# marekvinkler/NTrace

Measured on AMD Instinct MI355X. Metric: Mrays/sec (primary + 8xAO) on Crytek Sponza, higher is better.
Workload: dtype f32

## Files before the change

### ntrace_amd/csrc/ntr_api.cpp

```cpp

#include <hip/hip_runtime.h>

#include <cstdarg>
#include <cstdio>
#include <cstring>
#include <mutex>

#include "ntrace_amd.h"
#include "ntr_internal.h"
#include "compact_bvh.h"
#include "device_scratch.h"
#include "sched_state.h"
#include "trace_kernels.h"
#include "trace_plan.h"

namespace {

thread_local char g_err[512] = "";

}

namespace ntr {

int set_error(int code, const char* fmt, ...)
// ... 91 lines not shown
            if (zk != hipSuccess) return hip_fail(zk, "zero_words launch");
        }
        L->refresh = hs.refresh;
        hint->predicted = false;
        hint->uses++;
        if (hs.useOrder) p.order = hint->order;
        if (L->refresh) {
            const hipError_t ze = ntr_launch_zero_words(hint->cost, orderBlocks, s);
            if (ze != hipSuccess) return hip_fail(ze, "zero_words launch");
            p.cost = hint->cost;
        }
    }

    if (pl.predictable && !(hint && hint->valid) && !p.order) {
        rc = top_table_get(ds, p.nodes, nodesBytes, s, false, &L->predTable);
        if (rc != NTR_OK) return rc;
        rc = predict_scratch_get(ds, s, orderBlocks, &L->predScratch);
        if (rc != NTR_OK) return rc;
        if (L->predScratch) p.order = (hint && pl.hintable) ? hint->order : L->predScratch->order;
        else L->predTable = nullptr;
    }

    L->probeCoherence = !L->predScratch && hint && L->refresh && pl.probeOnRefresh;
    if (L->probeCoherence) {
        rc = top_table_get(ds, p.nodes, nodesBytes, s, false, &L->predTable);
        if (rc != NTR_OK) return rc;
    }
    const unsigned int* word = nullptr;
    if (L->predScratch) word = L->predScratch->classCount + NTR_SCHED_PRED_CLASSES + 2;
    else if (hint && pl.hintable && hint->numBlocks == orderBlocks && hint->order) word = hint->order + orderBlocks + 2;
    const bool routed = pl.coherentRoute == 1 && word != nullptr;
    L->persistentSide = variant == NTR_VARIANT_PERSISTENT || routed;
    L->perraySide = variant != NTR_VARIANT_PERSISTENT || routed;
    if ((pl.minipool && pl.poolKFromDevice) || L->persistentSide) p.poolK = word;

    TraceParams& pp = L->pp = p;
    if (L->persistentSide) {
        rc = counter_set_take(ds, capturing, &pp.counter);
        if (rc != NTR_OK) return rc;
        pp.numBlocks = pl.persistentBlocks; pp.numBlocksIncoherent = pl.numBlocksIncoherent; pp.numBlocksDivergent = pl.numBlocksDivergent;
        pp.fetchThreshold = pl.persistentFetchThreshold;
        pp.shardRays = pl.shardRays;
        if (pp.order) {
            pp.orderBlocks = orderBlocks;
            pp.shardRays = ((orderBlocks + pp.numHeads - 1) / pp.numHeads) * 256;
        }
        pp.routeSkip = routed ? NTR_ROUTE_SKIP_COHERENT : 0;
    }
    if (routed) {
        p.routeSkip = NTR_ROUTE_SKIP_INCOHERENT;
        if (variant == NTR_VARIANT_PERSISTENT) { p.fetchThreshold = pl.perrayFetchThreshold; p.poolKConst = 1; }
    }
    return NTR_OK;
}

static int launch_trace(DeviceState* ds, const Tunables& tun, const TracePlan& pl, const TraceLaunch& L, hipStream_t s, float* seconds,
                        NtrTraceStats* stats)
{
    const TraceParams& p = L.p;
    NtrSchedHint* hint = L.hint;
    const int orderBlocks = pl.orderBlocks;
    StreamEvents<2> ev(s);
    if (seconds) {
        NTR_HIP(ev.create());
        NTR_HIP(hipStreamSynchronize(s));
        NTR_HIP(ev.record(0));
    }
    if (L.predScratch) {
        const hipError_t pe = ntr_launch_predict(p.rays, p.numRays, orderBlocks, L.predTable->table, L.predTable->count, L.predScratch->classCount,
                                                 L.predScratch->classList, (hint && pl.hintable) ? hint->order : L.predScratch->order,
                                                 (hint && pl.hintable) ? hint->order + orderBlocks + 2 : nullptr, pl.minipoolWide, s);
        if (pe != hipSuccess) return hip_fail(pe, "predict launch");
    } else if (L.probeCoherence) {
        const hipError_t ce = ntr_launch_coherence(p.rays, p.numRays, orderBlocks, L.predTable->table, L.predTable->count, hint->order + orderBlocks,
                                                  pl.minipoolWide, s);
        if (ce != hipSuccess) return hip_fail(ce, "coherence launch");
    }
    hipError_t le = hipSuccess;
    if (L.persistentSide) {
        le = ntr_launch_zero_words(L.pp.counter, kPoolHeadsMax * 16, s);
        if (le != hipSuccess) return hip_fail(le, "zero_words launch");
        le = ntr_launch_trace(pl.persistentVariant, &L.pp, pl.persistentBlocks, s);
        if (le != hipSuccess) return hip_fail(le, "trace_bvh launch");
    }
    if (L.perraySide) {
        le = pl.variant == NTR_VARIANT_PERSISTENT ? ntr_launch_trace(NTR_VARIANT_PERRAY_UNIFIED_MINI, &p, pl.perrayBlocks, s)
                                                  : ntr_launch_trace(pl.launchVariant, &p, pl.launchBlocks, s);
        if (le != hipSuccess) return hip_fail(le, "trace_bvh launch");
    }
    if (seconds) NTR_HIP(ev.record(1));
    if (L.refresh) {
        le = ntr_launch_sched_order(hint->cost, orderBlocks, tun.schedClasses, hint->order, 1, s);
        if (le != hipSuccess) return hip_fail(le, "sched_order launch");
        hint->valid = true;
    }
    if (seconds) {
        float ms = 0.0f;
        NTR_HIP(ev.elapsed(0, 1, &ms));
        *seconds = ms * 1e-3f;
        unsigned int st = 0;
        const int rc = status_fetch(ds, s, &st);
        if (rc != NTR_OK) return rc;
        if (st & NTR_STATUS_STACK_OVERFLOW) return set_error(NTR_ERR_OVERFLOW, "trace_bvh: traversal stack overflow");
    }
    if (stats) {
        unsigned long long h[4];
        NTR_HIP(hipMemcpyAsync(h, ds->stats, sizeof(h), hipMemcpyDeviceToHost, s));
        NTR_HIP(hipStreamSynchronize(s));
        stats->numRays = p.numRays;
        stats->numInnerVisits = (int64_t)h[0]; stats->numTriTests = (int64_t)h[1]; stats->numLeafVisits = (int64_t)h[2]; stats->numHits = (int64_t)h[3];
    }
    return NTR_OK;
}

static int trace_impl(const char* kernelName, int32_t numRays, int32_t anyHit, const NtrRay* d_rays,
                      NtrRayResult* d_results, const void* d_nodes, int64_t nodesBytes, const void* d_triWoop,
                      int64_t triWoopBytes, const int32_t* d_triIndex, int32_t layout, uint32_t bvhFlags,
                      void* stream, float* seconds, NtrTraceStats* stats, NtrSchedHint* hint = nullptr)
{
    if (seconds) *seconds = 0.0f;
    if (stats) memset(stats, 0, sizeof(*stats));
    const KernelInfo* k = find_kernel(kernelName);
    if (!k) return set_error(NTR_ERR_UNKNOWN_KERNEL, "unknown kernel '%s'", kernelName ? kernelName : "(null)");
    if (numRays < 0) return set_error(NTR_ERR_INVALID, "ntr_trace_bvh: numRays < 0");
    if (numRays == 0) return NTR_OK;
    if (!d_nodes || !d_triWoop || !d_triIndex)
        return set_error(NTR_ERR_INVALID, "CudaBVHTracer: No BVH!");
    if (layout != k->cfg.bvhLayout)
        return set_error(NTR_ERR_LAYOUT, "CudaBVHTracer: Incorrect BVH layout!");
    if (!d_rays || !d_results) return set_error(NTR_ERR_INVALID, "ntr_trace_bvh: null ray/result buffer");
    int rc = check_nodes_bytes("ntr_trace_bvh", "node buffer size", nodesBytes);
    if (rc != NTR_OK) return rc;
    if (triWoopBytes < 16 || (triWoopBytes % 16) != 0 || triWoopBytes > 0xFFFFFFFFll)
        return set_error(NTR_ERR_INVALID, "ntr_trace_bvh: triWoop buffer size must be a multiple of 16 in [16, 4 GiB)");

    DeviceState* ds = nullptr;
    rc = current_device_state_ready(&ds);
    if (rc != NTR_OK) return rc;
    hipStream_t s = (hipStream_t)stream;

    const Tunables tun = tunables();
    const TraceBatchDesc bd = describe_batch(k, numRays, anyHit, (uint64_t)d_nodes, nodesBytes, (uint64_t)d_triWoop, triWoopBytes, bvhFlags,
                                             stats != nullptr, stream_is_capturing(s), hint != nullptr, ds->numCUs);
    const TracePlan pl = plan_trace(tun, bd);

    TraceLaunch L;
    TraceParams& p = L.p;
    p.numRays = numRays; p.anyHit = anyHit ? 1 : 0; p.rays = d_rays; p.results = d_results; p.bvhFlags = bvhFlags;
    p.nodes = d_nodes; p.woop = d_triWoop; p.triIndex = d_triIndex; p.nodesBytes = (uint32_t)nodesBytes; p.woopBytes = (uint32_t)triWoopBytes;
    p.status = ds->status; p.stats = ds->stats;
    p.numHeads = pl.numHeads; p.chunk = pl.chunk; p.fetchThreshold = pl.fetchThreshold; p.wholeWave = pl.wholeWave; p.prefetchAfter = pl.prefetchAfter;
    p.flatFetch = pl.flatFetch; p.uniformPrologue = pl.uniformPrologue; p.splitSlice = pl.splitSlice; p.leafSwitchBelow = pl.leafSwitchBelow;
    p.octant = pl.octant; p.poolKConst = pl.poolKConst;
    if (stats) NTR_HIP(hipMemsetAsync(ds->stats, 0, 4 * sizeof(unsigned long long), s));

    rc = bind_trace(ds, tun, pl, bd.capturing, nodesBytes, s, hint, &L);
    if (rc != NTR_OK) return rc;
    return launch_trace(ds, tun, pl, L, s, seconds, stats);
}

}

static int env_int(const char* name, int def)
{
    const char* v = getenv(name);
    return (v && *v) ? atoi(v) : def;
}

namespace ntr {
static Tunables g_tun;
static bool g_tunLoaded = false;
static std::mutex g_tunMu;

static void tunables_load_locked()
{
    Tunables t;
    t.chunk = env_int("NTR_TRACE_CHUNK", 64);
    t.fetchThreshold = env_int("NTR_TRACE_FETCH_THRESHOLD", -1);
    t.leafSwitchBelow = env_int("NTR_TRACE_LEAF_SWITCH", -1);
    t.blocksPerCU = env_int("NTR_TRACE_BLOCKS_PER_CU", 7);
    t.blocksPerCUIncoherent = env_int("NTR_TRACE_BLOCKS_PER_CU_INCOHERENT", 3);
    t.blocksPerCUDivergent = env_int("NTR_TRACE_BLOCKS_PER_CU_DIVERGENT", 4);
    t.octant = env_int("NTR_TRACE_OCTANT", 1);
    t.flatFetch = env_int("NTR_TRACE_FLAT_FETCH", 1);
    t.uniformPrologue = env_int("NTR_TRACE_UNIFORM_PROLOGUE", 1);
    t.splitSlice = env_int("NTR_TRACE_SPLIT_SLICE", 8);
    t.wholeWave = env_int("NTR_TRACE_WHOLE_WAVE", 1);
    t.prefetchAfter = env_int("NTR_TRACE_PREFETCH_AFTER", 8);
    t.minipool = env_int("NTR_TRACE_MINIPOOL", -1);
    t.minipoolWide = env_int("NTR_TRACE_MINIPOOL_WIDE", -1);
    t.minipoolThreshold = env_int("NTR_TRACE_MINIPOOL_THRESHOLD", 48);
    t.unified = env_int("NTR_TRACE_UNIFIED", 1);
    t.poolHeads = env_int("NTR_TRACE_POOL_HEADS", 128);
    t.autoHint = env_int("NTR_TRACE_AUTO_HINT", 1);
    t.autoHintMinRays = env_int("NTR_TRACE_AUTO_HINT_MIN_RAYS", 1 << 17);
    t.route = env_int("NTR_TRACE_ROUTE", 1);
    t.persistentHints = env_int("NTR_TRACE_PERSISTENT_HINTS", 1);
    t.predict = env_int("NTR_TRACE_PREDICT", 1);
    t.predictPersistent = env_int("NTR_TRACE_PREDICT_PERSISTENT", 1);
    t.predictDepth = env_int("NTR_TRACE_PREDICT_DEPTH", 9);
    t.predictMinRays = env_int("NTR_TRACE_PREDICT_MIN_RAYS", 1 << 20);
    t.predictMinNodes = env_int("NTR_TRACE_PREDICT_MIN_NODES", 4096);
    t.schedRefreshEvery = env_int("NTR_SCHED_REFRESH_EVERY", 16);
    t.schedClasses = env_int("NTR_SCHED_CLASSES", 32);
    t.lbvhSplit = env_int("NTR_LBVH_SPLIT", 3072);
    t.lbvhAggLds = env_int("NTR_LBVH_AGG_LDS", 1);
    t.lbvhSortItems = env_int("NTR_LBVH_SORT_ITEMS", 0);
    t.lbvhAggStaged = env_int("NTR_LBVH_AGG_STAGED", -1);
    if (t.chunk < 1) t.chunk = 1;
    g_tun = t;
    g_tunLoaded = true;
}

Tunables tunables()
{
    std::lock_guard<std::mutex> lk(g_tunMu);
    if (!g_tunLoaded) tunables_load_locked();
    return g_tun;
}
}

extern "C" int ntr_tunables_reload(void)
{
    std::lock_guard<std::mutex> lk(ntr::g_tunMu);
    ntr::tunables_load_locked();
    return NTR_OK;
}


using namespace ntr;

extern "C" {

const char* ntr_last_error(void) { return g_err; }
int ntr_version(void) { return 100; }

int ntr_device_count(int* count)
{
    if (!count) return set_error(NTR_ERR_INVALID, "ntr_device_count: null argument");
    hipError_t e = hipGetDeviceCount(count);
    if (e != hipSuccess) { *count = 0; return hip_fail(e, "hipGetDeviceCount"); }
    return NTR_OK;
}

int ntr_set_device(int device) { NTR_HIP(hipSetDevice(device)); return NTR_OK; }

int ntr_malloc(void** d_ptr, size_t bytes)
{
    if (!d_ptr) return set_error(NTR_ERR_INVALID, "ntr_malloc: null argument");
    *d_ptr = nullptr;
    if (bytes == 0) return NTR_OK;
    NTR_HIP(hipMalloc(d_ptr, bytes));
    return NTR_OK;
}

int ntr_free(void* d_ptr)
{
    if (d_ptr) NTR_HIP(hipFree(d_ptr));
    return NTR_OK;
}

int ntr_memcpy_h2d(void* d, const void* h, size_t n, void* stream)
{
    if (n == 0) return NTR_OK;
    NTR_HIP(hipMemcpyAsync(d, h, n, hipMemcpyHostToDevice, (hipStream_t)stream));
    NTR_HIP(hipStreamSynchronize((hipStream_t)stream));
    return NTR_OK;
}

int ntr_memcpy_d2h(void* h, const void* d, size_t n, void* stream)
{
    if (n == 0) return NTR_OK;
    NTR_HIP(hipMemcpyAsync(h, d, n, hipMemcpyDeviceToHost, (hipStream_t)stream));
    NTR_HIP(hipStreamSynchronize((hipStream_t)stream));
    return NTR_OK;
}

int ntr_memcpy_d2d(void* dst, const void* src, size_t n, void* stream)
{
    if (n == 0) return NTR_OK;
    NTR_HIP(hipMemcpyAsync(dst, src, n, hipMemcpyDeviceToDevice, (hipStream_t)stream));
    return NTR_OK;
}

int ntr_memset(void* d, int value, size_t n, void* stream)
{
    if (n == 0) return NTR_OK;
    NTR_HIP(hipMemsetAsync(d, value, n, (hipStream_t)stream));
    return NTR_OK;
}

int ntr_stream_synchronize(void* stream)
{
    NTR_HIP(hipStreamSynchronize((hipStream_t)stream));
    return NTR_OK;
}

int ntr_query_config(const char* kernelName, NtrKernelConfig* config)
{
    if (!config) return set_error(NTR_ERR_INVALID, "ntr_query_config: null config");
    const KernelInfo* k = find_kernel(kernelName);
    if (!k) {
        config->bvhLayout = NTR_BVHLayout_Max;
        config->blockWidth = config->blockHeight = config->usePersistentThreads = 0;
        return set_error(NTR_ERR_UNKNOWN_KERNEL, "unknown kernel '%s'", kernelName ? kernelName : "(null)");
    }
    *config = k->cfg;
    return NTR_OK;
}

int ntr_trace_bvh(const char* kernelName, int32_t numRays, int32_t anyHit, const NtrRay* d_rays,
                  NtrRayResult* d_results, const void* d_nodes, int64_t nodesBytes, const void* d_triWoop,
                  int64_t triWoopBytes, const int32_t* d_triIndex, int32_t layout, uint32_t bvhFlags, void* stream,
                  float* seconds)
{
    return trace_impl(kernelName, numRays, anyHit, d_rays, d_results, d_nodes, nodesBytes, d_triWoop, triWoopBytes,
                      d_triIndex, layout, bvhFlags, stream, seconds, nullptr);
}

int ntr_trace_bvh_hinted(const char* kernelName, int32_t numRays, int32_t anyHit, const NtrRay* d_rays,
                         NtrRayResult* d_results, const void* d_nodes, int64_t nodesBytes, const void* d_triWoop,
                         int64_t triWoopBytes, const int32_t* d_triIndex, int32_t layout, uint32_t bvhFlags, void* stream,
                         float* seconds, NtrSchedHint* hint)
{
    return trace_impl(kernelName, numRays, anyHit, d_rays, d_results, d_nodes, nodesBytes, d_triWoop, triWoopBytes,
                      d_triIndex, layout, bvhFlags, stream, seconds, nullptr, hint);
}

int ntr_trace_plan(const char* kernelName, int32_t numRays, int32_t anyHit, uint64_t nodesAddr, int64_t nodesBytes, uint64_t triWoopAddr,
                   int64_t triWoopBytes, uint32_t bvhFlags, int32_t numCUs, int32_t flags, NtrTracePlan* plan)
{
    if (!plan) return set_error(NTR_ERR_INVALID, "ntr_trace_plan: null plan");
    memset(plan, 0, sizeof(*plan));
    const KernelInfo* k = find_kernel(kernelName);
    if (!k) return set_error(NTR_ERR_UNKNOWN_KERNEL, "unknown kernel '%s'", kernelName ? kernelName : "(null)");
    if (numRays < 0 || numCUs < 1 || nodesBytes < 0 || triWoopBytes < 0) return set_error(NTR_ERR_INVALID, "ntr_trace_plan: bad argument");
    const TraceBatchDesc bd = describe_batch(k, numRays, anyHit, nodesAddr, nodesBytes, triWoopAddr, triWoopBytes, bvhFlags,
                                             (flags & NTR_PLAN_FLAG_STATS) != 0, (flags & NTR_PLAN_FLAG_CAPTURING) != 0,
// ... 200 lines not shown
```

### ntrace_amd/csrc/ntr_internal.h

```cpp
#pragma once
#include <hip/hip_runtime.h>

#include "ntrace_amd.h"

namespace ntr {
constexpr int kMaxDevices = 64;

int set_error(int code, const char* fmt, ...) __attribute__((format(printf, 2, 3)));
int hip_fail(hipError_t e, const char* what);

struct Tunables {
    int chunk, fetchThreshold, leafSwitchBelow, blocksPerCU, blocksPerCUIncoherent, blocksPerCUDivergent, poolHeads, octant, unified, flatFetch, uniformPrologue, splitSlice, wholeWave, prefetchAfter, minipool, minipoolThreshold, minipoolWide;
    int autoHint, autoHintMinRays, persistentHints, route, predict, predictPersistent, predictDepth, predictMinRays, predictMinNodes;
    int schedRefreshEvery, schedClasses;
    int lbvhSplit, lbvhAggLds, lbvhAggStaged, lbvhSortItems;
};
Tunables tunables();

bool stream_is_capturing(hipStream_t s);

size_t lbvh_sort_scratch_bytes(int n);
int lbvh_sort_codes(int n, const int32_t* d_tri, const float* d_pos, const float sceneMin[3], const float sceneMax[3], void* scratch,
                    hipStream_t s, const unsigned int** keys, const int** idx, const unsigned int** errWord);
}

extern "C" int ntr_top_table_refresh(const void* d_nodes, int64_t nodesBytes, void* stream);

#define NTR_HIP(call)                                            \
    do {                                                         \
        hipError_t _e = (call);                                  \
        if (_e != hipSuccess) return ::ntr::hip_fail(_e, #call); \
    } while (0)
```

### ntrace_amd/csrc/trace_kernels.h

```cpp
#pragma once
#include <hip/hip_runtime.h>
#include <stdint.h>

#include "ntrace_amd.h"

#ifndef NTR_TRACE_WAVES_PER_BLOCK
#define NTR_TRACE_WAVES_PER_BLOCK 4
#endif
#ifndef NTR_TRACE_MIN_WAVES_PER_SIMD
#define NTR_TRACE_MIN_WAVES_PER_SIMD 1
#endif
#ifndef NTR_TRACE_PERSISTENT_MIN_WAVES_PER_SIMD
#define NTR_TRACE_PERSISTENT_MIN_WAVES_PER_SIMD 1
#endif

#define NTR_VARIANT_PERRAY 0
#define NTR_VARIANT_PERSISTENT 1
#define NTR_VARIANT_PERRAY_STATS 2
#define NTR_VARIANT_PERSISTENT_UNIFIED 5
#define NTR_VARIANT_PERRAY_UNIFIED_W1 6
#define NTR_MINIPOOL_MAX_K 16
#define NTR_VARIANT_PERRAY_UNIFIED_MINI 7

#define NTR_ROUTE_SKIP_COHERENT 1
#define NTR_ROUTE_SKIP_INCOHERENT 2
#define NTR_BATCH_WORD_K(w) ((w) & 0xFFFFu)
#define NTR_BATCH_WORD_INCOHERENT(w) (NTR_BATCH_WORD_K(w) > 1u || ((w) & NTR_BATCH_DIVERGENT) != 0u)

#define NTR_STATUS_STACK_OVERFLOW 1u


namespace ntr {

struct TraceParams {
    int32_t numRays;
    int32_t anyHit;
    const NtrRay* rays;
    NtrRayResult* results;
    const void* nodes;
    const void* woop;
    uint32_t nodesBytes;
    uint32_t woopBytes;
    const int32_t* triIndex;
    int32_t* counter;
    unsigned int* status;
    int32_t chunk;
    int32_t shardRays;
    int32_t numHeads;
    int32_t numBlocks;
    int32_t numBlocksIncoherent;
    int32_t numBlocksDivergent;
    int32_t orderBlocks;
    int32_t fetchThreshold;
    int32_t wholeWave;
    int32_t prefetchAfter;
    uint32_t bvhFlags;
    int32_t leafSwitchBelow;
    int32_t octant;
    int32_t flatFetch;
    int32_t uniformPrologue;
    int32_t splitSlice;
    const unsigned int* order;
    unsigned int* cost;
    unsigned long long* stats;
    const unsigned int* poolK;
    int32_t poolKConst;
    int32_t routeSkip;
};

}

extern "C" hipError_t ntr_launch_trace(int variant, const ntr::TraceParams* p, int numBlocks, hipStream_t stream);
#define NTR_TOP_DEPTH_MAX 10
#define NTR_SCHED_PRED_CLASSES 64
#define NTR_SCHED_PRED_WORDS (NTR_SCHED_PRED_CLASSES + 3)
extern "C" hipError_t ntr_launch_top_table(const void* d_nodes, unsigned int nodesBytes, int depth, void* d_table,
                                           unsigned int* d_tableCount, hipStream_t stream);
extern "C" hipError_t ntr_launch_predict(const void* d_rays, int numRays, int numBlocks, const void* d_table,
                                         const unsigned int* d_tableCount, unsigned int* d_classCount, unsigned int* d_classList,
                                         unsigned int* d_order, unsigned int* d_poolKCopy, int poolKWide, hipStream_t stream);
extern "C" hipError_t ntr_launch_predict_costs(const void* d_rays, int numRays, int numBlocks, const void* d_table,
                                               const unsigned int* d_tableCount, unsigned int* d_blockCost, hipStream_t stream);
extern "C" hipError_t ntr_launch_coherence(const void* d_rays, int numRays, int numBlocks, const void* d_table, const unsigned int* d_tableCount,
                                           unsigned int* d_out, int poolKWide, hipStream_t stream);
extern "C" hipError_t ntr_launch_leaf_depth_level(const void* d_nodes, unsigned int nodesBytes, const void* d_woop, unsigned int woopVec4, const int* d_triIndex,
                                                  int numTris, const unsigned int* d_qin, const unsigned int* d_nIn, unsigned int* d_qout, unsigned int* d_nOut,
                                                  unsigned int capacity, unsigned int gridThreads, int depth, int* d_depthByTri, hipStream_t stream);
extern "C" hipError_t ntr_launch_secondary_block_costs(const void* d_inResults, int first, int count, int numSamples, const int* d_depthByTri, int numTris,
                                                       unsigned int* d_blockCost, hipStream_t stream);
extern "C" hipError_t ntr_launch_zero_words(void* d_ptr, int words, hipStream_t stream);
extern "C" hipError_t ntr_launch_status_exchange(unsigned int* d_status, unsigned int* d_out, hipStream_t stream);
extern "C" hipError_t ntr_launch_sched_order(const unsigned int* d_cost, int numBlocks, int classes, unsigned int* d_order,
                                             int keepIfAllZero, hipStream_t stream);
extern "C" hipError_t ntr_launch_identity_order(unsigned int* d_order, int numBlocks, hipStream_t stream);
extern "C" hipError_t ntr_launch_selftest_division(const float* d_x, const float* d_d, int nx, int nd,
                                                   unsigned int* d_mismatches, hipStream_t stream);
extern "C" hipError_t ntr_launch_selftest_division_hard(int xe0, int de0, unsigned long long* d_counts, hipStream_t stream);
```

### ntrace_amd/csrc/trace_kernels.hip

```cpp

#include <hip/hip_runtime.h>
#include <stdint.h>
#include <float.h>

#include "trace_kernels.h"
#include "trace_arith.h"

namespace ntr {

static constexpr int kSentinel = 0x76543210;
static constexpr int LDS_DEPTH = 16;
static constexpr int SPILL_DEPTH = 88;

typedef __amdgpu_buffer_rsrc_t Rsrc;
typedef unsigned int u32x4 __attribute__((ext_vector_type(4)));

__device__ __forceinline__ Rsrc make_rsrc(const void* p, unsigned int bytes)
{
    return __builtin_amdgcn_make_buffer_rsrc(const_cast<void*>(p), 0, (int)bytes, 0x00020000);
}
__device__ __forceinline__ float4 ld4(Rsrc r, int byteOfs)
{
    u32x4 v = __builtin_amdgcn_raw_buffer_load_b128(r, byteOfs, 0, 0);
    return make_float4(__uint_as_float(v.x), __uint_as_float(v.y), __uint_as_float(v.z), __uint_as_float(v.w));
// ... 166 lines not shown
        if (t > r.tmin && t < r.tmax) {
            const float u = dot4(u4, r.ox, r.oy, r.oz, 1.0f) + t * dot4(u4, r.dx, r.dy, r.dz, 0.0f);
            if (u >= 0.0f) {
                const float v = dot4(v4, r.ox, r.oy, r.oz, 1.0f) + t * dot4(v4, r.dx, r.dy, r.dz, 0.0f);
                if (v >= 0.0f && (u + v) <= 1.0f) { tt = t; uu = u; vv = v; }
            }
        }
        if (tt > r.tmin && tt < r.tmax) {
            r.tmax = tt;
            hitAddr = ofs >> 4;
            hitU = uu;
            hitV = vv;
            if (anyHit) return true;
        }
        if (nextWord == 0x80000000u) {
            if (STATS) ls.leaves++;
            break;
        }
    }
    return false;
}

__device__ __forceinline__ void store_result(NtrRayResult* __restrict__ results, const int* __restrict__ triIndex,
                                             int rayIdx, int hitAddr, float t, float u, float v)
{
    int4 out;
    out.x = (hitAddr < 0) ? -1 : triIndex[hitAddr];
    out.y = __float_as_int(t);
    out.z = (hitAddr < 0) ? 0 : __float_as_int(u);
    out.w = (hitAddr < 0) ? 0 : __float_as_int(v);
    reinterpret_cast<int4*>(results)[rayIdx] = out;
}

__device__ __forceinline__ void load_ray(const NtrRay* __restrict__ rays, int rayIdx, RayRegs& r)
{
    const float4 o = reinterpret_cast<const float4*>(rays)[rayIdx * 2 + 0];
    const float4 d = reinterpret_cast<const float4*>(rays)[rayIdx * 2 + 1];
    r.ox = o.x; r.oy = o.y; r.oz = o.z; r.tmin = o.w;
    r.dx = d.x; r.dy = d.y; r.dz = d.z; r.tmax = d.w;
    r.rx = exact_rcp(d.x); r.ry = exact_rcp(d.y); r.rz = exact_rcp(d.z);
}

template <bool FAST, bool STATS, bool DYNAMIC_FETCH, bool SLICED = false>
__device__ __forceinline__ void traverse(Rsrc nodes, Rsrc woop, RayRegs& r, int& node,
                                         LaneStack& st, int (&spill)[SPILL_DEPTH], bool anyHit,
                                         int& hitAddr, float& hitU, float& hitV, LaneStats& ls, unsigned int* status,
                                         bool poolEmpty, int fetchThreshold, int leafSwitchBelow, int& slice)
{
    unsigned long long live = __ballot(node != kSentinel);
    while (live != 0ull) {
        if (SLICED && --slice < 0) break;
        for (;;) {
            const bool inner = (unsigned)node < (unsigned)kSentinel;
            const unsigned long long innerMask = __ballot(inner);
            if (innerMask == 0ull) break;
            if (__popcll(innerMask) < leafSwitchBelow && __ballot(node < 0) != 0ull) break;
            inner_step<FAST>(nodes, inner, r, node, st, spill, status);
            if (STATS && inner) ls.inner++;
        }
        if (node < 0) {
            if (leaf_step<STATS>(woop, r, node, anyHit, hitAddr, hitU, hitV, ls)) node = kSentinel;
            else node = stack_pop(st, spill);
        }
        live = __ballot(node != kSentinel);
        if (DYNAMIC_FETCH && !poolEmpty && __popcll(live) < fetchThreshold) break;
    }
}
template <bool FAST, bool STATS, bool DYNAMIC_FETCH>
__device__ __forceinline__ void traverse(Rsrc nodes, Rsrc woop, RayRegs& r, int& node,
                                         LaneStack& st, int (&spill)[SPILL_DEPTH], bool anyHit,
                                         int& hitAddr, float& hitU, float& hitV, LaneStats& ls, unsigned int* status,
                                         bool poolEmpty, int fetchThreshold, int leafSwitchBelow)
{
    int never = 0;
    traverse<FAST, STATS, DYNAMIC_FETCH, false>(nodes, woop, r, node, st, spill, anyHit, hitAddr, hitU, hitV, ls, status, poolEmpty, fetchThreshold,
                                                leafSwitchBelow, never);
}

__device__ __forceinline__ u32x4 rsrc_words(const void* p, unsigned int bytes)
{
    const unsigned long long a = (unsigned long long)p;
    u32x4 w;
    w.x = __builtin_amdgcn_readfirstlane((unsigned int)a);
    w.y = __builtin_amdgcn_readfirstlane((unsigned int)(a >> 32) & 0xFFFFu);
    w.z = __builtin_amdgcn_readfirstlane(bytes);
    w.w = 0x00020000u;
    return w;
}

__device__ __forceinline__ void fetch64_two_buffers(u32x4 rsrcA, u32x4 rsrcB, int ofs, unsigned long long maskA,
                                                    unsigned long long maskB, float4& a, float4& b, float4& c, float4& d)
{
    u32x4 va, vb, vc, vd;
    unsigned long long sav;
    asm volatile(
        "s_mov_b64 %[sav], exec\n\t"
        "s_and_b64 exec, %[sav], %[ma]\n\t"
        "buffer_load_dwordx4 %[a], %[ofs], %[ra], 0 offen\n\t"
        "buffer_load_dwordx4 %[b], %[ofs], %[ra], 0 offen offset:16\n\t"
        "buffer_load_dwordx4 %[c], %[ofs], %[ra], 0 offen offset:32\n\t"
        "buffer_load_dwordx4 %[d], %[ofs], %[ra], 0 offen offset:48\n\t"
        "s_and_b64 exec, %[sav], %[mb]\n\t"
        "buffer_load_dwordx4 %[a], %[ofs], %[rb], 0 offen\n\t"
        "buffer_load_dwordx4 %[b], %[ofs], %[rb], 0 offen offset:16\n\t"
        "buffer_load_dwordx4 %[c], %[ofs], %[rb], 0 offen offset:32\n\t"
        "buffer_load_dwordx4 %[d], %[ofs], %[rb], 0 offen offset:48\n\t"
        "s_mov_b64 exec, %[sav]\n\t"
        "s_waitcnt vmcnt(0)"
        : [a] "=&v"(va), [b] "=&v"(vb), [c] "=&v"(vc), [d] "=&v"(vd), [sav] "=&s"(sav)
        : [ofs] "v"(ofs), [ra] "s"(rsrcA), [rb] "s"(rsrcB), [ma] "s"(maskA), [mb] "s"(maskB)
        : "memory", "scc");
    a = make_float4(__uint_as_float(va.x), __uint_as_float(va.y), __uint_as_float(va.z), __uint_as_float(va.w));
    b = make_float4(__uint_as_float(vb.x), __uint_as_float(vb.y), __uint_as_float(vb.z), __uint_as_float(vb.w));
    c = make_float4(__uint_as_float(vc.x), __uint_as_float(vc.y), __uint_as_float(vc.z), __uint_as_float(vc.w));
    d = make_float4(__uint_as_float(vd.x), __uint_as_float(vd.y), __uint_as_float(vd.z), __uint_as_float(vd.w));
}

__device__ __forceinline__ void fetch64_two_buffers_into(u32x4 rsrcA, u32x4 rsrcB, int ofs, unsigned long long maskA,
                                                         unsigned long long maskB, float4& a, float4& b, float4& c, float4& d)
{
    u32x4 va = {__float_as_uint(a.x), __float_as_uint(a.y), __float_as_uint(a.z), __float_as_uint(a.w)};
    u32x4 vb = {__float_as_uint(b.x), __float_as_uint(b.y), __float_as_uint(b.z), __float_as_uint(b.w)};
    u32x4 vc = {__float_as_uint(c.x), __float_as_uint(c.y), __float_as_uint(c.z), __float_as_uint(c.w)};
    u32x4 vd = {__float_as_uint(d.x), __float_as_uint(d.y), __float_as_uint(d.z), __float_as_uint(d.w)};
    unsigned long long sav;
    asm volatile(
        "s_mov_b64 %[sav], exec\n\t"
        "s_and_b64 exec, %[sav], %[ma]\n\t"
        "buffer_load_dwordx4 %[a], %[ofs], %[ra], 0 offen\n\t"
        "buffer_load_dwordx4 %[b], %[ofs], %[ra], 0 offen offset:16\n\t"
        "buffer_load_dwordx4 %[c], %[ofs], %[ra], 0 offen offset:32\n\t"
        "buffer_load_dwordx4 %[d], %[ofs], %[ra], 0 offen offset:48\n\t"
        "s_and_b64 exec, %[sav], %[mb]\n\t"
        "buffer_load_dwordx4 %[a], %[ofs], %[rb], 0 offen\n\t"
        "buffer_load_dwordx4 %[b], %[ofs], %[rb], 0 offen offset:16\n\t"
        "buffer_load_dwordx4 %[c], %[ofs], %[rb], 0 offen offset:32\n\t"
        "buffer_load_dwordx4 %[d], %[ofs], %[rb], 0 offen offset:48\n\t"
        "s_mov_b64 exec, %[sav]\n\t"
        "s_waitcnt vmcnt(0)"
        : [a] "+v"(va), [b] "+v"(vb), [c] "+v"(vc), [d] "+v"(vd), [sav] "=&s"(sav)
        : [ofs] "v"(ofs), [ra] "s"(rsrcA), [rb] "s"(rsrcB), [ma] "s"(maskA), [mb] "s"(maskB)
        : "memory", "scc");
    a = make_float4(__uint_as_float(va.x), __uint_as_float(va.y), __uint_as_float(va.z), __uint_as_float(va.w));
    b = make_float4(__uint_as_float(vb.x), __uint_as_float(vb.y), __uint_as_float(vb.z), __uint_as_float(vb.w));
    c = make_float4(__uint_as_float(vc.x), __uint_as_float(vc.y), __uint_as_float(vc.z), __uint_as_float(vc.w));
    d = make_float4(__uint_as_float(vd.x), __uint_as_float(vd.y), __uint_as_float(vd.z), __uint_as_float(vd.w));
}

struct UnifiedBufs {
    const char* nodes; const char* woop;
    unsigned int nodesBytes, woopBytes;
    u32x4 rNodes, rWoop;
    bool uniformPrologue;
    const char* base;
    unsigned int dN, dW;
    unsigned int limNode;
    int limTri;
};
__device__ __forceinline__ UnifiedBufs unified_bufs(const TraceParams& p)
{
    UnifiedBufs u;
    u.nodes = (const char*)p.nodes; u.woop = (const char*)p.woop;
    u.nodesBytes = p.nodesBytes; u.woopBytes = p.woopBytes;
    u.rNodes = rsrc_words(p.nodes, p.nodesBytes); u.rWoop = rsrc_words(p.woop, p.woopBytes);
    u.uniformPrologue = p.uniformPrologue != 0;
    const unsigned long long an = (unsigned long long)p.nodes, aw = (unsigned long long)p.woop;
    const unsigned long long lo = an < aw ? an : aw;
    u.base = (const char*)lo;
    u.dN = (unsigned int)(an - lo); u.dW = (unsigned int)(aw - lo);
    u.limNode = p.nodesBytes - 64u;
    u.limTri = ~(int)((p.woopBytes - 64u) >> 4);
    return u;
}

template <bool FLAT>
__device__ __forceinline__ void unified_fetch(const UnifiedBufs& ub, int node, float4& a, float4& b, float4& c, float4& d)
{
    const bool inner = (unsigned)node < (unsigned)kSentinel;
    const bool atTri = node < 0;
    if (FLAT) {
        asm volatile("" : "=v"(a.x), "=v"(a.y), "=v"(a.z), "=v"(a.w), "=v"(b.x), "=v"(b.y), "=v"(b.z), "=v"(b.w));
        asm volatile("" : "=v"(c.x), "=v"(c.y), "=v"(c.z), "=v"(c.w), "=v"(d.x), "=v"(d.y), "=v"(d.z), "=v"(d.w));
        const bool okNode = (unsigned)node <= ub.limNode, okTri = atTri && node >= ub.limTri;
        const bool flatOk = okNode || okTri;
        const unsigned int cofs = okNode ? ub.dN + (unsigned)node : ub.dW + ((unsigned)(~node) << 4);
        if (flatOk) {
            typedef const __attribute__((address_space(1))) u32x4* global_u4_ptr;
            const global_u4_ptr q = (global_u4_ptr)((const __attribute__((address_space(1))) char*)ub.base + cofs);
            const u32x4 qa = q[0], qb = q[1], qc = q[2], qd = q[3];
            a = make_float4(__uint_as_float(qa.x), __uint_as_float(qa.y), __uint_as_float(qa.z), __uint_as_float(qa.w));
            b = make_float4(__uint_as_float(qb.x), __uint_as_float(qb.y), __uint_as_float(qb.z), __uint_as_float(qb.w));
            c = make_float4(__uint_as_float(qc.x), __uint_as_float(qc.y), __uint_as_float(qc.z), __uint_as_float(qc.w));
            d = make_float4(__uint_as_float(qd.x), __uint_as_float(qd.y), __uint_as_float(qd.z), __uint_as_float(qd.w));
        }
        const unsigned long long odd = __ballot((inner || atTri) && !flatOk);
        if (odd != 0ull)
            fetch64_two_buffers_into(ub.rNodes, ub.rWoop, inner ? node : (~node) * 16, __ballot(inner && !flatOk), __ballot(atTri && !flatOk), a, b, c, d);
    } else {
        const int ofs = inner ? node : (~node) * 16;
        fetch64_two_buffers(ub.rNodes, ub.rWoop, ofs, __ballot(inner), __ballot(atTri), a, b, c, d);
    }
}

template <bool FAST, int OCT, int LD = LDS_DEPTH>
__device__ __forceinline__ void inner_advance(const float4& a, const float4& b, const float4& c, const float4& d, const RayRegs& r, int& node,
                                              LaneStack& st, int (&spill)[SPILL_DEPTH], unsigned int* status)
{
    float mn0, mx0, mn1, mx1;
    ray_box2<FAST, OCT>(r, a, b, c, mn0, mx0, mn1, mx1);
    const bool i0 = (mn0 <= mx0) && (mx0 >= r.tmin) && (mn0 <= r.tmax);
    const bool i1 = (mn1 <= mx1) && (mx1 >= r.tmin) && (mn1 <= r.tmax);
    const int c0 = __float_as_int(d.x), c1 = __float_as_int(d.y);
    const bool swp = i1 && (!i0 || mn0 > mn1);
    const int nearC = swp ? c1 : c0, farC = swp ? c0 : c1;
    if (i0 && i1) stack_push<LD>(st, spill, farC, status);
    node = (i0 || i1) ? nearC : stack_pop<LD>(st, spill);
}

template <bool FAST, int OCT, int LD = LDS_DEPTH>
__device__ __forceinline__ void unified_advance(const float4& a, const float4& b, const float4& c, const float4& d, RayRegs& r, int& node,
                                                LaneStack& st, int (&spill)[SPILL_DEPTH], bool anyHit, int& hitAddr, float& hitU, float& hitV,
                                                unsigned int* status)
{
    const bool inner = (unsigned)node < (unsigned)kSentinel;
    const bool atTri = node < 0;
    if (inner) {
        inner_advance<FAST, OCT, LD>(a, b, c, d, r, node, st, spill, status);
    } else if (atTri) {
        bool leafDone = __float_as_uint(a.x) == 0x80000000u;
        if (!leafDone) {
            const float Oz = a.w - r.ox * a.x - r.oy * a.y - r.oz * a.z;
            const float ooDz = 1.0f / dot4(a, r.dx, r.dy, r.dz, 0.0f);
            const float t = Oz * ooDz;
            float tt = FLT_MAX, uu = 0.0f, vv = 0.0f;
            if (t > r.tmin && t < r.tmax) {
                const float u = dot4(b, r.ox, r.oy, r.oz, 1.0f) + t * dot4(b, r.dx, r.dy, r.dz, 0.0f);
                if (u >= 0.0f) {
                    const float v = dot4(c, r.ox, r.oy, r.oz, 1.0f) + t * dot4(c, r.dx, r.dy, r.dz, 0.0f);
                    if (v >= 0.0f && (u + v) <= 1.0f) { tt = t; uu = u; vv = v; }
                }
            }
            bool terminated = false;
            if (tt > r.tmin && tt < r.tmax) {
                r.tmax = tt;
                hitAddr = ~node;
                hitU = uu;
                hitV = vv;
                terminated = anyHit;
            }
            if (terminated) node = kSentinel;
            else if (__float_as_uint(d.x) == 0x80000000u) leafDone = true;
            else node -= 3;
        }
        if (leafDone) node = stack_pop<LD>(st, spill);
    }
}

typedef float f32x4 __attribute__((ext_vector_type(4)));
typedef const __attribute__((address_space(4))) f32x4* const_f32x4_ptr;

template <bool FAST, int OCT>
__device__ __forceinline__ void uniform_prologue(const UnifiedBufs& ub, const RayRegs& r, int& node, LaneStack& st, int (&spill)[SPILL_DEPTH],
                                                 unsigned int* status)
{
    if ((reinterpret_cast<unsigned long long>(ub.nodes) & 63ull) != 0ull) return;
    for (;;) {
        const bool live = node != kSentinel;
        const unsigned long long liveMask = __ballot(live);
        if (liveMask == 0ull) return;
        const int unode = __builtin_amdgcn_readlane(node, (int)__builtin_ctzll(liveMask));
        if (__ballot(live && node != unode) != 0ull) return;
        if ((unsigned)unode >= (unsigned)kSentinel || (unsigned)unode > ub.nodesBytes - 64u) return;
        const const_f32x4_ptr q = (const_f32x4_ptr)(ub.nodes + (unsigned)unode);
        const f32x4 A = q[0], B = q[1], C = q[2], D = q[3];
        if (live)
            inner_advance<FAST, OCT>(make_float4(A.x, A.y, A.z, A.w), make_float4(B.x, B.y, B.z, B.w), make_float4(C.x, C.y, C.z, C.w),
                                     make_float4(D.x, D.y, D.z, D.w), r, node, st, spill, status);
    }
}

template <bool FAST, bool FLAT, int OCT, bool PROLOGUE, bool SLICED>
__device__ __forceinline__ void traverse_unified(const UnifiedBufs& ub, RayRegs& r, int& node, LaneStack& st,
                                                 int (&spill)[SPILL_DEPTH], bool anyHit, int& hitAddr, float& hitU, float& hitV,
                                                 unsigned int* status, bool poolEmpty, int fetchThreshold, int& slice)
{
    if (PROLOGUE && ub.uniformPrologue) uniform_prologue<FAST, OCT>(ub, r, node, st, spill, status);
    for (;;) {
        const unsigned long long live = __ballot(node != kSentinel);
        if (live == 0ull) break;
        if (!poolEmpty && __popcll(live) < fetchThreshold) break;
        if (SLICED && --slice < 0) break;
        float4 a, b, c, d;
        unified_fetch<FLAT>(ub, node, a, b, c, d);
        if (FLAT) { keep(a); keep(b); keep(c); keep(d); }
        unified_advance<FAST, OCT>(a, b, c, d, r, node, st, spill, anyHit, hitAddr, hitU, hitV, status);
    }
}
template <bool FAST, bool FLAT, int OCT = 8, bool PROLOGUE = false>
__device__ __forceinline__ void traverse_unified(const UnifiedBufs& ub, RayRegs& r, int& node, LaneStack& st,
                                                 int (&spill)[SPILL_DEPTH], bool anyHit, int& hitAddr, float& hitU, float& hitV,
                                                 unsigned int* status, bool poolEmpty, int fetchThreshold)
{
    int never = 0;
    traverse_unified<FAST, FLAT, OCT, PROLOGUE, false>(ub, r, node, st, spill, anyHit, hitAddr, hitU, hitV, status, poolEmpty, fetchThreshold, never);
}

}
#include "trace_split.h"
namespace ntr {

template <bool FLATF>
__device__ __forceinline__ void minipool_body(const TraceParams& p, unsigned int K, lds_int* stackBase);

#define NTR_PERRAY_BOUNDS(W) __launch_bounds__((W) * 64, NTR_TRACE_MIN_WAVES_PER_SIMD)
template <int WAVES, bool STATS, bool UNIFIED = false, bool FLATF = true, bool MINI = false>
__device__ __forceinline__ void perray_body(const TraceParams& p)
{
    __shared__ int s_stack[WAVES][LDS_DEPTH][64];
    if constexpr (MINI) {
        static_assert(WAVES == 1 && UNIFIED && !STATS, "the mini-pool shares the one-wave unified-step launch");
        unsigned int K = (unsigned int)p.poolKConst;
        if (p.poolK) {
            const unsigned int word = *p.poolK;
            if (p.routeSkip == NTR_ROUTE_SKIP_INCOHERENT && NTR_BATCH_WORD_INCOHERENT(word)) return;
            K = NTR_BATCH_WORD_K(word);
        }
        bool pooled = K >= 2u && K <= (unsigned int)NTR_MINIPOOL_MAX_K;
        if (pooled) {
            minipool_body<FLATF>(p, K, (lds_int*)&s_stack[0][0][threadIdx.x]);
            return;
        }
    }
    const int lane = threadIdx.x & 63, wave = threadIdx.x >> 6;
    constexpr int PARTS = 4 / WAVES;
    const unsigned int g = blockIdx.x / PARTS, part = blockIdx.x % PARTS;
    const unsigned int block = p.order ? p.order[g] : g;
    const int rayIdx = block * 256 + part * (WAVES * 64) + threadIdx.x;
    const bool valid = rayIdx < p.numRays;
    const Rsrc nodes = make_rsrc(p.nodes, p.nodesBytes), woop = make_rsrc(p.woop, p.woopBytes);

    unsigned long long tl0 = 0;
    if (p.cost) tl0 = __builtin_amdgcn_s_memrealtime();

    RayRegs r;
    load_ray(p.rays, valid ? rayIdx : 0, r);
    LaneStack st;
    int spill[SPILL_DEPTH];
    st.lds = (lds_int*)&s_stack[wave][0][lane];
    NTR_STACK_RESET(st);

    int hitAddr = -1;
    float hitU = 0.0f, hitV = 0.0f;
    int node = (valid && r.tmin < r.tmax) ? 0 : kSentinel;
    LaneStats ls = {0u, 0u, 0u};

    const bool fastWave = (p.bvhFlags & NTR_BVH_FASTDIV) && __ballot(node != kSentinel && !ray_is_nice(r, p.bvhFlags)) == 0ull;
    int oct = 8;
    if (UNIFIED && fastWave && p.octant && (p.bvhFlags & NTR_BVH_ORDERED)) {
        const unsigned long long liveMask = __ballot(node != kSentinel);
        const unsigned long long sx = __ballot(node != kSentinel && r.dx < 0.0f), sy = __ballot(node != kSentinel && r.dy < 0.0f),
                                 sz = __ballot(node != kSentinel && r.dz < 0.0f);
        if ((sx == 0ull || sx == liveMask) && (sy == 0ull || sy == liveMask) && (sz == 0ull || sz == liveMask))
            oct = (sx ? 1 : 0) | (sy ? 2 : 0) | (sz ? 4 : 0);
    }
    if (UNIFIED) {
        const UnifiedBufs ub = unified_bufs(p);
#define NTR_UNIFIED_OCT(O) traverse_unified<true, FLATF, O, true>(ub, r, node, st, spill, p.anyHit != 0, hitAddr, hitU, hitV, p.status, true, 0)
        if (oct < 8) {
            switch (oct) {
                case 0: NTR_UNIFIED_OCT(0); break;
                case 1: NTR_UNIFIED_OCT(1); break;
                case 2: NTR_UNIFIED_OCT(2); break;
                case 3: NTR_UNIFIED_OCT(3); break;
                case 4: NTR_UNIFIED_OCT(4); break;
                case 5: NTR_UNIFIED_OCT(5); break;
                case 6: NTR_UNIFIED_OCT(6); break;
                default: NTR_UNIFIED_OCT(7); break;
            }
        }
#undef NTR_UNIFIED_OCT
        else if (fastWave) traverse_unified<true, FLATF, 8, true>(ub, r, node, st, spill, p.anyHit != 0, hitAddr, hitU, hitV, p.status, true, 0);
        else traverse_unified<false, FLATF, 8, true>(ub, r, node, st, spill, p.anyHit != 0, hitAddr, hitU, hitV, p.status, true, 0);
    } else if (fastWave) traverse<true, STATS, false>(nodes, woop, r, node, st, spill, p.anyHit != 0, hitAddr, hitU, hitV, ls, p.status, true, 0, p.leafSwitchBelow);
    else traverse<false, STATS, false>(nodes, woop, r, node, st, spill, p.anyHit != 0, hitAddr, hitU, hitV, ls, p.status, true, 0, p.leafSwitchBelow);

    if (p.cost && lane == 0)
        atomicMax(&p.cost[block], (unsigned int)(__builtin_amdgcn_s_memrealtime() - tl0));
    if (!valid) return;
    store_result(p.results, p.triIndex, rayIdx, hitAddr, r.tmax, hitU, hitV);
    if (STATS) {
        atomicAdd(&p.stats[0], (unsigned long long)ls.inner);
        atomicAdd(&p.stats[1], (unsigned long long)ls.tris);
        atomicAdd(&p.stats[2], (unsigned long long)ls.leaves);
        atomicAdd(&p.stats[3], (unsigned long long)(hitAddr >= 0));
    }
}

template <int WAVES, bool STATS, bool UNIFIED = false, bool FLATF = true>
__global__ NTR_PERRAY_BOUNDS(WAVES) void trace_bvh_perray(TraceParams p)
{
    perray_body<WAVES, STATS, UNIFIED, FLATF, false>(p);
}
#define NTR_MINI_BOUNDS __launch_bounds__(64)
__global__ NTR_MINI_BOUNDS void trace_bvh_perray_mini(TraceParams p)
{
    perray_body<1, false, true, true, true>(p);
}
__global__ NTR_MINI_BOUNDS void trace_bvh_perray_mini_desc(TraceParams p)
{
    perray_body<1, false, true, false, true>(p);
}

template <int WAVES, bool UNIFIED = false, bool FLATF = true>
__global__ __launch_bounds__(WAVES * 64, NTR_TRACE_PERSISTENT_MIN_WAVES_PER_SIMD) void trace_bvh_persistent(TraceParams p)
{
    __shared__ int s_stack[WAVES][LDS_DEPTH][64];
    const int lane = threadIdx.x & 63, wave = threadIdx.x >> 6;
    const Rsrc nodes = make_rsrc(p.nodes, p.nodesBytes), woop = make_rsrc(p.woop, p.woopBytes);
    const bool anyHit = p.anyHit != 0;
    const bool bvhFast = (p.bvhFlags & NTR_BVH_FASTDIV) != 0;
    int numBlocksEff = p.numBlocks;
    const unsigned int batchWord = p.poolK ? *p.poolK : 1u;
    const bool incoherentBatch = NTR_BATCH_WORD_INCOHERENT(batchWord);
    if (p.routeSkip == NTR_ROUTE_SKIP_COHERENT && !incoherentBatch) return;
    const int gridIncoherent = NTR_BATCH_WORD_K(batchWord) > 1u ? p.numBlocksIncoherent : p.numBlocksDivergent;
    if (incoherentBatch && gridIncoherent > 0 && gridIncoherent < numBlocksEff) numBlocksEff = gridIncoherent;
    if ((int)blockIdx.x >= numBlocksEff) return;

    LaneStack st;
    int spill[SPILL_DEPTH];
    st.lds = (lds_int*)&s_stack[wave][0][lane];
    st.sp = 0;
    st.tos = kSentinel;

    RayRegs r = {0, 0, 0, 0, 0, 0, 0, 0, 0, 0, 0};
    int node = kSentinel, rayIdx = -1, hitAddr = -1;
    float hitU = 0.0f, hitV = 0.0f;
    bool nice = true;
    int chunkNext = 0, chunkEnd = 0;
// ... 249 lines not shown
```

Baseline: 15890.

## Add certain-step shortcut in uniform prologue using origin containment masks

In the wave-uniform prologue, when every live ray has tmin of zero, the ray's segment extent is bounded conservatively. Scalar-vs-vector compare masks test whether each ray origin lies inside exactly one child box and its whole segment cannot reach the other child. If all live lanes fit that case, they step straight to the containing child with no full slab test and no stack push. This targets the top-of-tree traversal cost for AO rays, which is on by default only for any-hit rays. It adds inline-assembly exec-mask code and a give-up counter, and when the test fails it costs extra work.

```diff
diff --git a/ntrace_amd/csrc/ntr_api.cpp b/ntrace_amd/csrc/ntr_api.cpp
--- a/ntrace_amd/csrc/ntr_api.cpp
+++ b/ntrace_amd/csrc/ntr_api.cpp
@@ -267,6 +267,7 @@
     p.numHeads = pl.numHeads; p.chunk = pl.chunk; p.fetchThreshold = pl.fetchThreshold; p.wholeWave = pl.wholeWave; p.prefetchAfter = pl.prefetchAfter;
     p.flatFetch = pl.flatFetch; p.uniformPrologue = pl.uniformPrologue; p.splitSlice = pl.splitSlice; p.leafSwitchBelow = pl.leafSwitchBelow;
     p.octant = pl.octant; p.poolKConst = pl.poolKConst;
+    p.certainSteps = (tun.certainSteps >= 2 || (tun.certainSteps == 1 && anyHit)) ? 1 : 0;
     if (stats) NTR_HIP(hipMemsetAsync(ds->stats, 0, 4 * sizeof(unsigned long long), s));
 
     rc = bind_trace(ds, tun, pl, bd.capturing, nodesBytes, s, hint, &L);
@@ -299,6 +300,7 @@
     t.octant = env_int("NTR_TRACE_OCTANT", 1);
     t.flatFetch = env_int("NTR_TRACE_FLAT_FETCH", 1);
     t.uniformPrologue = env_int("NTR_TRACE_UNIFORM_PROLOGUE", 1);
+    t.certainSteps = env_int("NTR_TRACE_CERTAIN_STEPS", 1);
     t.splitSlice = env_int("NTR_TRACE_SPLIT_SLICE", 8);
     t.wholeWave = env_int("NTR_TRACE_WHOLE_WAVE", 1);
     t.prefetchAfter = env_int("NTR_TRACE_PREFETCH_AFTER", 8);
diff --git a/ntrace_amd/csrc/ntr_internal.h b/ntrace_amd/csrc/ntr_internal.h
--- a/ntrace_amd/csrc/ntr_internal.h
+++ b/ntrace_amd/csrc/ntr_internal.h
@@ -10,7 +10,7 @@
 int hip_fail(hipError_t e, const char* what);
 
 struct Tunables {
-    int chunk, fetchThreshold, leafSwitchBelow, blocksPerCU, blocksPerCUIncoherent, blocksPerCUDivergent, poolHeads, octant, unified, flatFetch, uniformPrologue, splitSlice, wholeWave, prefetchAfter, minipool, minipoolThreshold, minipoolWide;
+    int chunk, fetchThreshold, leafSwitchBelow, blocksPerCU, blocksPerCUIncoherent, blocksPerCUDivergent, poolHeads, octant, unified, flatFetch, uniformPrologue, certainSteps, splitSlice, wholeWave, prefetchAfter, minipool, minipoolThreshold, minipoolWide;
     int autoHint, autoHintMinRays, persistentHints, route, predict, predictPersistent, predictDepth, predictMinRays, predictMinNodes;
     int schedRefreshEvery, schedClasses;
     int lbvhSplit, lbvhAggLds, lbvhAggStaged, lbvhSortItems;
diff --git a/ntrace_amd/csrc/trace_kernels.h b/ntrace_amd/csrc/trace_kernels.h
--- a/ntrace_amd/csrc/trace_kernels.h
+++ b/ntrace_amd/csrc/trace_kernels.h
@@ -59,6 +59,7 @@
     int32_t octant;
     int32_t flatFetch;
     int32_t uniformPrologue;
+    int32_t certainSteps;
     int32_t splitSlice;
     const unsigned int* order;
     unsigned int* cost;
diff --git a/ntrace_amd/csrc/trace_kernels.hip b/ntrace_amd/csrc/trace_kernels.hip
--- a/ntrace_amd/csrc/trace_kernels.hip
+++ b/ntrace_amd/csrc/trace_kernels.hip
@@ -342,6 +342,7 @@
     unsigned int nodesBytes, woopBytes;
     u32x4 rNodes, rWoop;
     bool uniformPrologue;
+    bool certainSteps;
     const char* base;
     unsigned int dN, dW;
     unsigned int limNode;
@@ -354,6 +355,7 @@
     u.nodesBytes = p.nodesBytes; u.woopBytes = p.woopBytes;
     u.rNodes = rsrc_words(p.nodes, p.nodesBytes); u.rWoop = rsrc_words(p.woop, p.woopBytes);
     u.uniformPrologue = p.uniformPrologue != 0;
+    u.certainSteps = p.certainSteps != 0 && (p.bvhFlags & NTR_BVH_ORDERED) != 0;
     const unsigned long long an = (unsigned long long)p.nodes, aw = (unsigned long long)p.woop;
     const unsigned long long lo = an < aw ? an : aw;
     u.base = (const char*)lo;
@@ -449,11 +451,106 @@
 typedef float f32x4 __attribute__((ext_vector_type(4)));
 typedef const __attribute__((address_space(4))) f32x4* const_f32x4_ptr;
 
-template <bool FAST, int OCT>
+static constexpr int kCertainGiveUpAfter = 2;
+
+__device__ __forceinline__ float certain_reach(float tmax, float d)
+{
+    const float p = tmax * fabsf(d);
+    return (p >= 0x1p-100f) ? p * 0x1.00001p0f : __builtin_inff();
+}
+template <int SIGN>
+__device__ __forceinline__ float certain_end(float o, float reach)
+{
+    const float s = SIGN > 0 ? o + reach : o - reach;
+    return __builtin_fmaf(fabsf(s), SIGN > 0 ? 0x1p-22f : -0x1p-22f, s);
+}
+
+__device__ __forceinline__ void certain_masks(f32x4 A, f32x4 B, f32x4 C, const RayRegs& r, float loX, float hiX, float loY, float hiY, float loZ,
+                                              float hiZ, unsigned long long live, unsigned long long& in0, unsigned long long& in1,
+                                              unsigned long long& reach)
+{
+    unsigned long long sav;
+    asm volatile(
+        "s_mov_b64 %[sav], exec\n\t"
+        "s_and_b64 exec, %[sav], %[live]\n\t"
+        "v_cmpx_le_f32 vcc, %[ax], %[ox]\n\t"
+        "v_cmpx_ge_f32 vcc, %[ay], %[ox]\n\t"
+        "v_cmpx_le_f32 vcc, %[az], %[oy]\n\t"
+        "v_cmpx_ge_f32 vcc, %[aw], %[oy]\n\t"
+        "v_cmpx_le_f32 vcc, %[cx], %[oz]\n\t"
+        "v_cmpx_ge_f32 vcc, %[cy], %[oz]\n\t"
+        "s_mov_b64 %[in0], exec\n\t"
+        "s_and_b64 exec, %[sav], %[live]\n\t"
+        "s_andn2_b64 exec, exec, %[in0]\n\t"
+        "s_cbranch_execz .Lcs_a%=\n\t"
+        "v_cmpx_le_f32 vcc, %[bx], %[ox]\n\t"
+        "v_cmpx_ge_f32 vcc, %[by], %[ox]\n\t"
+        "v_cmpx_le_f32 vcc, %[bz], %[oy]\n\t"
+        "v_cmpx_ge_f32 vcc, %[bw], %[oy]\n\t"
+        "v_cmpx_le_f32 vcc, %[cz], %[oz]\n\t"
+        "v_cmpx_ge_f32 vcc, %[cw], %[oz]\n\t"
+        "s_cbranch_execz .Lcs_a%=\n\t"
+        "s_mov_b64 %[in1], exec\n\t"
+        "v_cmpx_le_f32 vcc, %[ax], %[hx]\n\t"
+        "v_cmpx_ge_f32 vcc, %[ay], %[lx]\n\t"
+        "v_cmpx_le_f32 vcc, %[az], %[hy]\n\t"
+        "v_cmpx_ge_f32 vcc, %[aw], %[ly]\n\t"
+        "v_cmpx_le_f32 vcc, %[cx], %[hz]\n\t"
+        "v_cmpx_ge_f32 vcc, %[cy], %[lz]\n\t"
+        "s_mov_b64 %[reach], exec\n\t"
+        "s_branch .Lcs_b%=\n"
+        ".Lcs_a%=:\n\t"
+        "s_mov_b64 %[in1], 0\n\t"
+        "s_mov_b64 %[reach], 0\n"
+        ".Lcs_b%=:\n\t"
+        "s_mov_b64 exec, %[in0]\n\t"
+        "s_cbranch_execz .Lcs_c%=\n\t"
+        "v_cmpx_le_f32 vcc, %[bx], %[hx]\n\t"
+        "v_cmpx_ge_f32 vcc, %[by], %[lx]\n\t"
+        "v_cmpx_le_f32 vcc, %[bz], %[hy]\n\t"
+        "v_cmpx_ge_f32 vcc, %[bw], %[ly]\n\t"
+        "v_cmpx_le_f32 vcc, %[cz], %[hz]\n\t"
+        "v_cmpx_ge_f32 vcc, %[cw], %[lz]\n\t"
+        "s_or_b64 %[reach], %[reach], exec\n"
+        ".Lcs_c%=:\n\t"
+        "s_mov_b64 exec, %[sav]"
+        : [sav] "=&s"(sav), [in0] "=&s"(in0), [in1] "=&s"(in1), [reach] "=&s"(reach)
+        : [live] "s"(live), [ax] "s"(A.x), [ay] "s"(A.y), [az] "s"(A.z), [aw] "s"(A.w), [bx] "s"(B.x), [by] "s"(B.y), [bz] "s"(B.z), [bw] "s"(B.w),
+          [cx] "s"(C.x), [cy] "s"(C.y), [cz] "s"(C.z), [cw] "s"(C.w), [ox] "v"(r.ox), [oy] "v"(r.oy), [oz] "v"(r.oz), [lx] "v"(loX), [hx] "v"(hiX),
+          [ly] "v"(loY), [hy] "v"(hiY), [lz] "v"(loZ), [hz] "v"(hiZ)
+        : "vcc", "scc");
+}
+__device__ __forceinline__ void take_children(int& node, int c0, int c1, unsigned long long m0, unsigned long long m1)
+{
+    unsigned long long sav;
+    asm volatile(
+        "s_mov_b64 %[sav], exec\n\t"
+        "s_mov_b64 exec, %[m1]\n\t"
+        "v_mov_b32 %[node], %[c1]\n\t"
+        "s_mov_b64 exec, %[m0]\n\t"
+        "v_mov_b32 %[node], %[c0]\n\t"
+        "s_mov_b64 exec, %[sav]"
+        : [sav] "=&s"(sav), [node] "+v"(node)
+        : [m0] "s"(m0), [m1] "s"(m1), [c0] "s"(c0), [c1] "s"(c1));
+}
+
+template <bool FAST, int OCT, bool CERTAIN = false>
 __device__ __forceinline__ void uniform_prologue(const UnifiedBufs& ub, const RayRegs& r, int& node, LaneStack& st, int (&spill)[SPILL_DEPTH],
                                                  unsigned int* status)
 {
     if ((reinterpret_cast<unsigned long long>(ub.nodes) & 63ull) != 0ull) return;
+    bool tryCertain = false;
+    int uncertain = 0;
+    float loX = 0.0f, hiX = 0.0f, loY = 0.0f, hiY = 0.0f, loZ = 0.0f, hiZ = 0.0f;
+    if (CERTAIN && FAST) {
+        tryCertain = ub.certainSteps && __ballot(node != kSentinel && r.tmin != 0.0f) == 0ull;
+        if (tryCertain) {
+            const float fx = certain_reach(r.tmax, r.dx), fy = certain_reach(r.tmax, r.dy), fz = certain_reach(r.tmax, r.dz);
+            loX = r.dx < 0.0f ? certain_end<-1>(r.ox, fx) : r.ox; hiX = r.dx < 0.0f ? r.ox : certain_end<1>(r.ox, fx);
+            loY = r.dy < 0.0f ? certain_end<-1>(r.oy, fy) : r.oy; hiY = r.dy < 0.0f ? r.oy : certain_end<1>(r.oy, fy);
+            loZ = r.dz < 0.0f ? certain_end<-1>(r.oz, fz) : r.oz; hiZ = r.dz < 0.0f ? r.oz : certain_end<1>(r.oz, fz);
+        }
+    }
     for (;;) {
         const bool live = node != kSentinel;
         const unsigned long long liveMask = __ballot(live);
@@ -463,6 +560,16 @@
         if ((unsigned)unode >= (unsigned)kSentinel || (unsigned)unode > ub.nodesBytes - 64u) return;
         const const_f32x4_ptr q = (const_f32x4_ptr)(ub.nodes + (unsigned)unode);
         const f32x4 A = q[0], B = q[1], C = q[2], D = q[3];
+        if (CERTAIN && FAST && tryCertain) {
+            unsigned long long in0, in1, reach;
+            certain_masks(A, B, C, r, loX, hiX, loY, hiY, loZ, hiZ, liveMask, in0, in1, reach);
+            if ((in0 | in1) == liveMask && reach == 0ull) {
+                take_children(node, __float_as_int(D.x), __float_as_int(D.y), in0, in1);
+                uncertain = 0;
+                continue;
+            }
+            if (++uncertain >= kCertainGiveUpAfter) tryCertain = false;
+        }
         if (live)
             inner_advance<FAST, OCT>(make_float4(A.x, A.y, A.z, A.w), make_float4(B.x, B.y, B.z, B.w), make_float4(C.x, C.y, C.z, C.w),
                                      make_float4(D.x, D.y, D.z, D.w), r, node, st, spill, status);
@@ -474,7 +581,7 @@
                                                  int (&spill)[SPILL_DEPTH], bool anyHit, int& hitAddr, float& hitU, float& hitV,
                                                  unsigned int* status, bool poolEmpty, int fetchThreshold, int& slice)
 {
-    if (PROLOGUE && ub.uniformPrologue) uniform_prologue<FAST, OCT>(ub, r, node, st, spill, status);
+    if (PROLOGUE && ub.uniformPrologue) uniform_prologue<FAST, OCT, true>(ub, r, node, st, spill, status);
     for (;;) {
         const unsigned long long live = __ballot(node != kSentinel);
         if (live == 0ull) break;
```

Measured after the change: 16480 (median of 6 runs). 1.04x the previous value.
